# ruchikachavhan/diffusion-models-moe

Measured on AMD Instinct MI355X. Metric: images/sec SD-1.4 512² 50-step DDIM, expert mask on; 1→8 GPU scaling, higher is better.
Workload: dtype fp16; 1 GPU; SD-1.4 MoE-fied (relu, top-k 0.2, expert 20) + RemoveExperts skilled-expert mask, 512^2 (4x64x64 latents), 50 DDIM steps, CFG 7.5; prompts_per_gpu=8, global_batch=8, parallelism=dp1

## Files before the change

diffusion-models-moe_amd/csrc/gemm.hip:

```cpp
#include <array>
#include <utility>

#include "tune.h"
#include "../../include/sdmoe.h"
#include "gemm_kernel.h"

namespace {

enum TileId { T128x160, T64x160, T256x320, T256x160_42, T256x320_42, T128x320, T128x160_42, T64x320, T128x32, T128x64,
              T128x128, T64x128, NTILE };
struct TileShape { int bm, bn, wmw, wnw; };
constexpr TileShape kTile[NTILE] = {{128, 160, 2, 2}, {64, 160, 2, 2}, {256, 320, 2, 4}, {256, 160, 4, 2},
                                    {256, 320, 4, 2}, {128, 320, 2, 4}, {128, 160, 4, 2}, {64, 320, 2, 4},
                                    {128, 32, 2, 2},  {128, 64, 2, 2},  {128, 128, 2, 2}, {64, 128, 2, 2}};
struct Plan {
  int mode;
  int tile;
  int bk, stages;
  int ksplit;
  int kchunk;
  int kchunk2;
  int mfast;
};
struct TileRule { int tile, ks_want, stages_want; };
// ... 198 lines not shown
  const int pm = masked ? MODE_GEMM : mode;
  const TileRule r = choose_tile(pm, p);
  const int ksplit = plan_split(kTile[r.tile], pm, p, ws, ws_floats, r.ks_want);
  return tile_plan(mode, masked ? masked_tile(mode, r.tile, p) : r.tile, p, ksplit, r.stages_want);
}

bool plan_sets(int mode, const GemmParams& p, int rows_per_img, bool ws, long ws_floats, Plan* pl) {
  *pl = plan_launch(mode, p, ws, ws_floats);
  if (rows_per_img % kTile[pl->tile].bm == 0) return true;
  if (rows_per_img % 64) return false;
  const int tile = p.N % 160 == 0 ? T64x160 : T64x128;
  *pl = tile_plan(mode, tile, p, plan_split(kTile[tile], MODE_GEMM, p, ws, ws_floats, 0), 0);
  return true;
}

Plan plan_conv(const GemmParams& p, bool ws, long ws_floats) {
  Plan pl;
  if (plan_halo(p, ws, ws_floats, false, &pl)) return pl;
  return plan_launch(p.upsample ? MODE_CONV_UP : MODE_CONV, p, ws, ws_floats);
}

template <int MODE, int TILE>
int launch_kernel(const Plan& pl, const GemmParams& p, dim3 grid, hipStream_t s) {
  constexpr TileShape t = kTile[TILE];
  constexpr int NTH = 64 * t.wmw * t.wnw;
  if constexpr (!built(MODE, TILE)) return SDMOE_EUNSUP;
  else if constexpr (mode_halo(MODE)) gemm_kernel<t.bm, t.bn, t.wmw, t.wnw, MODE, 4, 32><<<grid, NTH, 0, s>>>(p);
  else if constexpr (!fits3(t, MODE)) gemm_kernel<t.bm, t.bn, t.wmw, t.wnw, MODE, 2, 64><<<grid, NTH, 0, s>>>(p);
  else if (pl.stages == 2) gemm_kernel<t.bm, t.bn, t.wmw, t.wnw, MODE, 2, 64><<<grid, NTH, 0, s>>>(p);
  else gemm_kernel<t.bm, t.bn, t.wmw, t.wnw, MODE, 3, 64><<<grid, NTH, 0, s>>>(p);
// ... 4 lines not shown
using LaunchFn = int (*)(const Plan&, const GemmParams&, dim3, hipStream_t);
template <int... KEY>
constexpr std::array<LaunchFn, sizeof...(KEY)> launch_table(std::integer_sequence<int, KEY...>) {
  return {{&launch_kernel<KEY / NTILE, KEY % NTILE>...}};
}
constexpr auto kLaunch = launch_table(std::make_integer_sequence<int, NMODE * NTILE>{});

int launch(const Plan& pl, GemmParams p, float* ws, hipStream_t s) {
  const TileShape& t = kTile[pl.tile];
  if (p.w_bstride && p.rows_per_batch % t.bm) return SDMOE_EUNSUP;
  if (p.image_set && p.rows_per_batch % t.bm) return SDMOE_EUNSUP;
  if (pl.ksplit > 1 && !ws) return SDMOE_EARG;
  p.ksplit = pl.ksplit; p.kchunk = pl.kchunk; p.kchunk2 = pl.kchunk2; p.mfast = pl.mfast;
  p.part = pl.ksplit > 1 ? ws : nullptr;
  p.diag = knob(KNOB_DIAG); p.res16 = knob(KNOB_RES16);
  const int direct = knob(KNOB_EPI_DIRECT);
  p.epi_direct = direct == 2 || (direct == 1 && p.R == nullptr);
  const dim3 grid(((p.M + t.bm - 1) / t.bm) * ((p.N + t.bn - 1) / t.bn) * pl.ksplit);
  if (const int st = kLaunch[pl.mode * NTILE + pl.tile](pl, p, grid, s)) return st;
  SDMOE_CHECK_LAUNCH();
  if (pl.ksplit > 1) {
    long nchunk = (long)p.M * (p.N / 8);
    int g = (int)((nchunk + 255) / 256);
    if (g > 2048) g = 2048;
    splitk_reduce_kernel<<<g, 256, 0, s>>>(p);
    SDMOE_CHECK_LAUNCH();
  }
  return SDMOE_OK;
}



// ... 435 lines not shown
                                long coladd_bstride, const void* R, long ldr, const void* X2, long ldx2, int Cin2,
                                void* Y, long ldy, int Cout, float* workspace, long workspace_floats, void* stream) {
  if (nimg == 0) return SDMOE_OK;
  if (!X || !gn_scale || !gn_shift || !Wt || !Y || nimg < 0 || H <= 0 || W <= 0 || Cout <= 0 || Cin2 < 0) return SDMOE_EARG;
  if (Cin % 64 || Cin2 % 64 || Cout % 8 || ldx % 8 || ldy % 8 || (R && ldr % 8) || (X2 && ldx2 % 8)) return SDMOE_ESHAPE;
  if ((X2 != nullptr) != (Cin2 > 0) || (X2 && R)) return SDMOE_EARG;
  GemmParams p{};
  conv_shape(p, nimg, H, W, Cin, Cin2, Cout, 1, 0, ACT_NONE);
  Plan pl;
  if (!plan_halo(p, workspace, workspace_floats, true, &pl)) return SDMOE_EUNSUP;
  if (const int st = fill_conv(p, X, ldx, Wt, bias, coladd, coladd_bstride, R, ldr, X2, ldx2, Y, ldy)) return st;
  p.gn_scale = gn_scale; p.gn_shift = gn_shift; p.gn_silu = silu;
  return launch(pl, p, workspace, (hipStream_t)stream);
}

extern "C" int sdmoe_groupnorm_apply(const void* X, long ldx, int nimg, int HW, int C, const float* scale,
                                     const float* shift, int silu, void* Y, long ldy, void* stream) {
  if (!X || !Y || !scale || !shift || nimg <= 0 || HW <= 0 || C <= 0) return SDMOE_EARG;
  if (C % 8 || ldx % 8 || ldy % 8) return SDMOE_ESHAPE;
  const long rows = (long)nimg * HW;
  gn_apply_kernel<<<grid_for(rows * (C / 8)), 256, 0, (hipStream_t)stream>>>(
      (const half_t*)X, ldx, HW, C, scale, shift, silu, (half_t*)Y, ldy, rows);
  SDMOE_CHECK_LAUNCH();
  return SDMOE_OK;
}

extern "C" int sdmoe_wmask_kmajor(const void* bits, long ldb, int N, int K, const int* perm, void* out, void* stream) {
  if (N == 0) return SDMOE_OK;
  if (!bits || !out || N < 0 || K <= 0) return SDMOE_EARG;
  if (K % 64 || ldb < K / 8) return SDMOE_ESHAPE;
// ... 16 lines not shown
```

diffusion-models-moe_amd/csrc/gemm_kernel.h:

```cpp
#pragma once
#include <type_traits>
#include <utility>
#include "common.h"

namespace {

typedef __attribute__((address_space(3))) void lds_void_t;

struct GemmParams {
  const half_t* A; long lda;
  const half_t* W; long ldw;
  const half_t* bias;
  const half_t* coladd; long coladd_bstride;
  const half_t* R; long ldr;
  half_t* C; long ldc;
  float* part;
  int M, N, K;
  int act;
  int rows_per_batch;
  int H, Wd, Cin, OH, OW, stride, upsample;
  int ksplit, kchunk;
  int kchunk2;
  int mfast;
  int a_bytes, w_bytes;
// ... 5 lines not shown
  const uint8_t* keep;
  int keep_bytes;
  const uint8_t* wmask;
  int wmask_bytes;
  const int* image_set;
  long wset_bytes;
  const float* ln_wsum;
  const float* ln_bias;
  float ln_eps;
  const half_t* A2; long lda2;
  int a2_bytes;
  long w_bstride;
  const float* colf; long colf_bstride;
  const half_t* gelu_tab;
  const float* gn_scale; const float* gn_shift; int gn_silu;
};

constexpr unsigned OOB = 0x80000000u;

SDMOE_DEV void bld16(__amdgpu_buffer_rsrc_t rs, char* lds_dst, unsigned voff, unsigned soff) {
  __builtin_amdgcn_raw_ptr_buffer_load_lds(rs, (lds_void_t*)lds_dst, 16, voff, soff, 0, 0);
}
SDMOE_DEV void wave_sync() {
  __builtin_amdgcn_fence(__ATOMIC_RELEASE, "wavefront");
  __builtin_amdgcn_wave_barrier();
  __builtin_amdgcn_fence(__ATOMIC_ACQUIRE, "wavefront");
}
template <int N>
SDMOE_DEV void vm_wait() { asm volatile("s_waitcnt vmcnt(%0)" ::"n"(N) : "memory"); }
SDMOE_DEV void vm_wait(int n) {
// ... 800 lines not shown
    for (int c = tid; c < BN; c += L.NT) {
      const bool ok = n0 + c < p.N;
      ln_col[c] = ok ? p.ln_wsum[n0 + c] : 0.f;
      ln_col[BN + c] = ok ? p.ln_bias[n0 + c] : 0.f;
    }
  }
  __syncthreads();
  constexpr int CPR = L.WN / 8;
  if (!G::GEGLU && p.act == ACT_NONE && (!p.R || p.res16 != 0)) {
    half4 b4[L.FN];
#pragma unroll
    for (int j = 0; j < L.FN; ++j) {
      const int n = nw + 16 * j + 4 * fg;
      b4[j] = (!G::LN && p.bias && n < p.N) ? *reinterpret_cast<const half4*>(p.bias + n) : (half4){0, 0, 0, 0};
    }
    if (!G::WKEEP && p.epi_direct) {
      const bool res = p.R != nullptr;
#pragma unroll
      for (int i = 0; i < L.FM; ++i) {
        __builtin_amdgcn_sched_barrier(0);
        const int m = mw + 16 * i + fr;
        const half_t* cap = (p.coladd && m < p.M) ? p.coladd + (long)(m / p.rows_per_batch) * p.coladd_bstride : nullptr;
        const float* cfp = (p.colf && m < p.M) ? p.colf + (long)(m / p.rows_per_batch) * p.colf_bstride : nullptr;
        float a = 0.f, c = 0.f;
        if constexpr (G::LN) {
          const int rl = wr * L.WM + 16 * i + fr;
          a = ln_row[2 * rl];
          c = ln_row[2 * rl + 1];
        }
        auto frag16 = [&](int j) -> uint2v {
          const int n = nw + 16 * j + 4 * fg;
          float4v v = acc[i][j];
// ... 22 lines not shown
          return __builtin_bit_cast(uint2v, y);
        };
#pragma unroll
        for (int j = 0; j + 1 < L.FN; j += 2) {
          const uint2v ya = frag16(j), yb = frag16(j + 1);
          const auto s0 = __builtin_amdgcn_permlane16_swap(ya[0], yb[0], false, false);
          const auto s1 = __builtin_amdgcn_permlane16_swap(ya[1], yb[1], false, false);
          const int n = nw + 16 * (j + (fg & 1)) + 8 * (fg >> 1);
          half8 o = __builtin_bit_cast(half8, (uint4v){s0[0], s1[0], s0[1], s1[1]});
          if (m < p.M && n < p.N) {
            if (res) {
              const half8 rr = *reinterpret_cast<const half8*>(p.R + (long)m * p.ldr + n);
#pragma unroll
              for (int r = 0; r < 8; ++r) o[r] = (half_t)((float)o[r] + (float)rr[r]);
            }
            if (p.diag & 8) asm volatile("" ::"v"(o));
            else *reinterpret_cast<half8*>(p.C + (long)m * p.ldc + n) = o;
          }
        }
        if constexpr (L.FN % 2) {
          const int n = nw + 16 * (L.FN - 1) + 4 * fg;
          half4 o = __builtin_bit_cast(half4, frag16(L.FN - 1));
          if (m < p.M && n < p.N) {
            if (res) {
              const half4 rr = *reinterpret_cast<const half4*>(p.R + (long)m * p.ldr + n);
#pragma unroll
              for (int r = 0; r < 4; ++r) o[r] = (half_t)((float)o[r] + (float)rr[r]);
            }
            if (p.diag & 8) asm volatile("" ::"v"(o));
            else *reinterpret_cast<half4*>(p.C + (long)m * p.ldc + n) = o;
          }
        }
      }
      return;
    }
    half_t* st = reinterpret_cast<half_t*>(smem) + wave * (L.WM / L.NPASS16) * L.RS16;
    constexpr int NCH16 = (L.WM / L.NPASS16) * CPR, NIT16 = (NCH16 + 63) / 64;
    const bool res = p.R != nullptr;
#pragma unroll
    for (int h = 0; h < L.NPASS16; ++h) {
      half8 rr[NIT16];
      if (res) {
#pragma unroll
        for (int it = 0; it < NIT16; ++it) {
          const int id = lane + 64 * it;
          const int r = id / CPR, c8 = id - r * CPR;
          const int m = mw + h * (L.WM / L.NPASS16) + r, n = nw + c8 * 8;
          rr[it] = (id < NCH16 && m < p.M && n < p.N) ? *reinterpret_cast<const half8*>(p.R + (long)m * p.ldr + n)
                                                      : (half8){0, 0, 0, 0, 0, 0, 0, 0};
        }
      }
#pragma unroll
      for (int i = 0; i < L.FM / L.NPASS16; ++i) {
// ... 35 lines not shown
          for (int r = 0; r < 4; ++r) y[r] = (half_t)v[r];
          *reinterpret_cast<half4*>(st + (16 * i + fr) * L.RS16 + 16 * j + 4 * fg) = y;
        }
      }
      wave_sync();
#pragma unroll
      for (int it = 0; it < NIT16; ++it) {
        const int id = lane + 64 * it;
        const int r = id / CPR, c8 = id - r * CPR;
        const int m = mw + h * (L.WM / L.NPASS16) + r, n = nw + c8 * 8;
        if (id >= NCH16 || m >= p.M || n >= p.N) continue;
        half8 o = *reinterpret_cast<const half8*>(st + r * L.RS16 + c8 * 8);
        if (res) {
#pragma unroll
          for (int j = 0; j < 8; ++j) o[j] = (half_t)((float)o[j] + (float)rr[it][j]);
        }
        if (p.diag & 8) asm volatile("" ::"v"(o));
        else *reinterpret_cast<half8*>(p.C + (long)m * p.ldc + n) = o;
      }
      wave_sync();
    }
    return;
  }
  if constexpr (G::GEGLU) {
    int lane_o = lane;
    asm volatile("" : "+v"(lane_o));
    const int fr_e = lane_o & 15, fg_e = lane_o >> 4;
    typedef _Float16 h2 __attribute__((ext_vector_type(2)));
    constexpr int NH = L.WN / 2;
    constexpr int FPP = L.FM % 2 == 0 ? 2 : 1;
    constexpr int RG = 16 * FPP;
    constexpr int GST = L.NW * 2 * RG * NH * 2;
    static_assert(NH % 8 == 0, "whole 16-B product chunks per row");
    static_assert(GST + L.NW * L.WN * 4 <= L.SMEM1, "GEGLU staging and bias must fit in the kernel's LDS");
    static_assert(GST + L.NW * L.WN * 4 == L.G_STAGING, "GEGLU staging size as the layout states it");
// ... 129 lines not shown
```

diffusion-models-moe_amd/csrc/norm.hip:

```cpp
#include "common.h"
#include "tune.h"
#include "../../include/sdmoe.h"

namespace {

constexpr int GN_SMALL_HW = 1024;
constexpr int GN_FUSED_HW = 256;

int gn_chunk_width(int C, int groups) {
  const int cpg = C / groups;
  int wc = cpg;
  while (wc % 8) wc += cpg;
  while (wc < 80 && C % (2 * wc) == 0 && 2 * wc <= 256) wc *= 2;
  return (wc <= 256 && wc / cpg <= 32 && C % wc == 0) ? wc : 0;
}

SDMOE_DEV float gn_ref(const half_t* g0, int cpg) {
  float s = 0.f;
#pragma unroll
  for (int j = 0; j < 8; ++j) s += (float)g0[(j * cpg) >> 3];
  return (float)(half_t)(s * 0.125f);
}

SDMOE_DEV void gn_accum8(const half8& v, const float (&rf)[8], float (&s1)[8], float (&s2)[8]) {
// ... 325 lines not shown
  const double n = (double)HW * cpg;
  const double ref = (double)gn_ref(X + (long)img * HW * ldx + g * cpg, cpg);
  const double m1 = a / n;
  double var = b / n - m1 * m1;
  if (var < 0) var = 0;
  const float mean = (float)(ref + m1);
  const float rstd = (float)(1.0 / sqrt(var + (double)eps));
  for (int c = lane; c < cpg; c += 64) {
    const int ch = g * cpg + c;
    const float sc = rstd * (float)gamma[ch];
    scale[(long)img * C + ch] = sc;
    shift[(long)img * C + ch] = (float)beta[ch] - mean * sc;
  }
}


template <int CPL>
__global__ __launch_bounds__(256) void layernorm_kernel(const half_t* __restrict__ X, long ldx, half_t* __restrict__ Y,
                                                        long ldy, int M, int C, const half_t* __restrict__ gamma,
                                                        const half_t* __restrict__ beta, float eps) {
  const int lane = threadIdx.x & 63, sub = lane & 7;
  const int row = blockIdx.x * (int)(blockDim.x >> 3) + (int)(threadIdx.x >> 3);
  const bool live = row < M;
  const half_t* xr = X + (long)(live ? row : 0) * ldx;
  half8 v[CPL];
#pragma unroll
  for (int i = 0; i < CPL; ++i) v[i] = *reinterpret_cast<const half8*>(xr + (sub + 8 * i) * 8);
  float s = 0.f;
#pragma unroll
  for (int i = 0; i < CPL; ++i)
// ... 54 lines not shown
  else
    gn_partial_kernel<1><<<dim3(S, nimg), 256, 0, s>>>((const half_t*)X, ldx, HW, C, groups, S, part);
  SDMOE_CHECK_LAUNCH();
  gn_finalize_kernel<<<dim3(groups, nimg), 64, 0, s>>>((const half_t*)X, ldx, HW, C, groups, S, part,
                                                       (const half_t*)gamma, (const half_t*)beta, eps, scale, shift);
  SDMOE_CHECK_LAUNCH();
  return SDMOE_OK;
}
}

extern "C" int sdmoe_groupnorm_stats(const void* X, long ldx, int nimg, int HW, int C, int groups,
                                     const void* gamma, const void* beta, float eps, float* scale, float* shift,
                                     float* workspace, long workspace_floats, void* stream) {
  return groupnorm_impl(X, ldx, nimg, HW, C, groups, gamma, beta, eps, scale, shift, workspace, workspace_floats,
                        stream);
}

extern "C" int sdmoe_groupnorm(const void* X, long ldx, int nimg, int HW, int C, int groups, const void* gamma,
                               const void* beta, float eps, int silu, void* Y, long ldy, float* scale, float* shift,
                               float* workspace, long workspace_floats, void* stream) {
  if (!Y || ldy % 8) return Y ? SDMOE_ESHAPE : SDMOE_EARG;
  if (knob(KNOB_GN_FUSED) && HW <= GN_FUSED_HW && X && gamma && beta && nimg > 0 && groups > 0 && C % groups == 0 &&
      C % 8 == 0 && ldx % 8 == 0 && groups <= 64) {
    const int wc = gn_chunk_width(C, groups);
    if (wc) {
      const int nchunk = C / wc;
      int S = (512 + nchunk * nimg - 1) / (nchunk * nimg);
      const int R = 256 / (wc / 8);
      if (S > HW / R) S = HW / R;
      if (S < 1) S = 1;
// ... 46 lines not shown
```

diffusion-models-moe_amd/sdmoe/_lib.py:

```python
from __future__ import annotations

import ctypes
import os

_HERE = os.path.dirname(os.path.abspath(__file__))
LIB_PATH = os.path.join(_HERE, "libsdmoe_hip.so")

_P = ctypes.c_void_p
_L = ctypes.c_long
_I = ctypes.c_int
_F = ctypes.c_float
_FP = ctypes.POINTER(ctypes.c_float)
_IP = ctypes.POINTER(ctypes.c_int)

SIGNATURES = {
    "sdmoe_linear": [_P, _L, _P, _L, _P, _P, _L, _I, _P, _L, _P, _L, _I, _I, _I, _I, _P, _L, _P],
    "sdmoe_conv3x3": [_P, _L, _I, _I, _I, _I, _P, _P, _P, _L, _P, _L, _P, _L, _I, _I, _I, _I, _P, _L, _P],
    "sdmoe_conv3x3_sc": [_P, _L, _I, _I, _I, _I, _P, _P, _P, _L, _P, _L, _I, _P, _L, _I, _I, _P, _L, _P],
    "sdmoe_conv3x3_gn": [_P, _L, _I, _I, _I, _I, _P, _P, _I, _P, _P, _P, _L, _P, _L, _P, _L, _I, _P, _L, _I, _P, _L,
                         _P],
    "sdmoe_groupnorm_apply": [_P, _L, _I, _I, _I, _P, _P, _I, _P, _L, _P],
    "sdmoe_mask_weight": [_P, _P, _L, _L, _P, _P],
    "sdmoe_groupnorm_stats": [_P, _L, _I, _I, _I, _I, _P, _P, _F, _P, _P, _P, _L, _P],
    "sdmoe_groupnorm": [_P, _L, _I, _I, _I, _I, _P, _P, _F, _I, _P, _L, _P, _P, _P, _L, _P],
    "sdmoe_gn_fold": [_P, _L, _I, _I, _P, _P, _P, _I, _P, _P, _P],
    "sdmoe_linear_per_image": [_P, _L, _P, _L, _L, _P, _L, _I, _P, _L, _P, _L, _I, _I, _I, _P, _L, _P],
    "sdmoe_layernorm": [_P, _L, _P, _L, _I, _I, _P, _P, _F, _P],
    "sdmoe_ln_fold": [_P, _L, _I, _I, _P, _P, _P, _P, _L, _P, _P, _P],
    "sdmoe_linear_ln": [_P, _L, _P, _L, _P, _P, _F, _P, _L, _I, _I, _I, _P],
    "sdmoe_linear_geglu_ln": [_P, _L, _P, _L, _P, _P, _F, _P, _L, _I, _I, _I, _I, _P, _L, _I, _P],
    "sdmoe_attention": [_P, _L, _P, _L, _P, _L, _P, _L, _I, _I, _I, _I, _I, _F, _P],
    "sdmoe_geglu_route": [_P, _L, _I, _I, _I, _I, _I, _P, _P, _P, _P, _P, _L, _P, _L, _P, _P, _P],
    "sdmoe_linear_geglu": [_P, _L, _P, _L, _P, _P, _L, _I, _I, _I, _I, _P, _L, _I, _P],
    "sdmoe_moe_topk_mask": [_P, _L, _I, _I, _I, _I, _I, _P, _L, _P, _P, _P],
    "sdmoe_moe_topk_keep": [_I, _I, _I, _I, _I, _P, _L, _P, _P, _P, _P],
# ... 107 lines not shown
```

diffusion-models-moe_amd/sdmoe/ops.py:

```python
from __future__ import annotations

import ctypes
import os

import torch

from . import _lib

ACT_NONE, ACT_SILU, ACT_GELU, ACT_RELU, ACT_QUICK_GELU = 0, 1, 2, 3, 4
ACT_BY_NAME = {"none": ACT_NONE, "silu": ACT_SILU, "gelu": ACT_GELU, "relu": ACT_RELU, "quick_gelu": ACT_QUICK_GELU}


_raw_stream = getattr(torch._C, "_cuda_getCurrentRawStream", None)
_cur_dev = getattr(torch._C, "_cuda_getDevice", None)


def _stream():
    if _raw_stream is not None and _cur_dev is not None:
        return _raw_stream(_cur_dev())
    return torch.cuda.current_stream().cuda_stream


def _ptr(t):
    return None if t is None else t.data_ptr()
# ... 347 lines not shown

def conv3x3_gn_launch(xp, ldx, nimg, H, W, Cin, w, bias, coladd, coladd_bstride, rp, ldr, out, op, ldy, Cout, gn,
                      sc=None):
    lib = _lib.load()
    ws = _workspace(out.device)
    x2p, ldx2, Cin2 = sc if sc is not None else (None, 0, 0)
    st = lib.sdmoe_conv3x3_gn(xp, ldx, nimg, H, W, Cin, gn[0].data_ptr(), gn[1].data_ptr(), int(bool(gn[2])),
                              _dev(w, "w"), _ptr(bias), _ptr(coladd), coladd_bstride, rp, ldr, x2p, ldx2, Cin2, op, ldy,
                              Cout, ws.data_ptr(), ws.numel(), _stream())
    if st == -3:
        return None
    _lib.check(st, "sdmoe_conv3x3_gn")
    return out


def conv3x3_launch(xp, ldx, nimg, H, W, Cin, w, bias, coladd, coladd_bstride, rp, ldr, out, op, ldy, Cout, stride,
                   upsample, act, sc=None):
    lib = _lib.load()
    ws = _workspace(out.device)
    if sc is not None:
        st = lib.sdmoe_conv3x3_sc(xp, ldx, nimg, H, W, Cin, _dev(w, "w"), _ptr(bias), _ptr(coladd), coladd_bstride,
                                  sc[0], sc[1], sc[2], op, ldy, Cout, act, ws.data_ptr(), ws.numel(), _stream())
        _lib.check(st, "sdmoe_conv3x3_sc")
        return out
    st = lib.sdmoe_conv3x3(xp, ldx, nimg, H, W, Cin, _dev(w, "w"), _ptr(bias), _ptr(coladd), coladd_bstride, rp, ldr,
                           op, ldy, Cout, stride, int(bool(upsample)), act, ws.data_ptr(), ws.numel(), _stream())
    _lib.check(st, "sdmoe_conv3x3")
    return out


# ... 585 lines not shown
```

diffusion-models-moe_amd/sdmoe/unet.py:

```python
from __future__ import annotations

import os

import torch
import torch.nn as nn
import torch.nn.functional as F

from . import ops
from .config import UNetConfig

CTX_LEN = 77
FUSED_GEGLU = True
FUSED_KEEP = True
FUSED_LN = os.environ.get("SDMOE_FUSED_LN", "1") != "0"
FUSED_LN_FFN = os.environ.get("SDMOE_FUSED_LN_FFN", "0") == "1"
FUSED_SC = os.environ.get("SDMOE_FUSED_SC", "1") != "0"
FUSED_GN = os.environ.get("SDMOE_FUSED_GN", "1") != "0"
GN_FOLD_MIN_HW = 1024
IN_PAD = 64
OUT_PAD = 8


def _buf(t):
    return nn.Parameter(t, requires_grad=False)


class LoRACompatibleLinear(nn.Module):

    def __init__(self, weight, bias=None):
        super().__init__()
        self.weight = _buf(weight)
        self.bias = None if bias is None else _buf(bias)
        self._sdmoe_deferred = 0
# ... 23 lines not shown
        self.weight = _buf(weight)
        self.bias = _buf(bias)
        self.stride = stride


class Norm(nn.Module):
    def __init__(self, weight, bias, eps, groups=None):
        super().__init__()
        self.weight = _buf(weight)
        self.bias = _buf(bias)
        self.eps = eps
        self.groups = groups

    def stats(self, x2d, nimg, HW):
        return ops.groupnorm_stats(x2d, nimg, HW, self.weight, self.bias, self.eps, self.groups)

    def normalize(self, x2d, nimg, HW, silu):
        return ops.groupnorm(x2d, nimg, HW, self.weight, self.bias, self.eps, self.groups, silu)


def act_code(fn):
    from_name = getattr(fn, "_sdmoe_act", None)
    if from_name is not None:
        return ops.ACT_BY_NAME[from_name]
    if fn is F.gelu or fn is torch.nn.functional.gelu:
        return ops.ACT_GELU
    if fn is F.relu or fn is torch.relu:
        return ops.ACT_RELU
    raise NotImplementedError(f"GEGLU activation {fn!r} has no HIP kernel (supported: gelu, relu)")

# ... 298 lines not shown
        n = ops.layernorm(hs, self.norm2.weight, self.norm2.bias, self.norm2.eps)
        hs = self.attn2.run(n, nimg, N, residual=hs, ctx2d=ctx2d)
        n = ops.layernorm(hs, self.norm3.weight, self.norm3.bias, self.norm3.eps)
        return self.ff.run(n, nimg, residual=hs)


class Transformer2DModel(nn.Module):

    def __init__(self, norm, proj_in, blocks, proj_out):
        super().__init__()
        self.norm = norm
        self.proj_in = proj_in
        self.transformer_blocks = nn.ModuleList(blocks)
        self.proj_out = proj_out

    def run(self, x, nimg, HW, ctx2d, out):
        pi = self.proj_in
        if FUSED_GN and HW >= GN_FOLD_MIN_HW and HW % 256 == 0 and x.shape[1] % 64 == 0 and not pi._forward_hooks:
            scale, shift = self.norm.stats(x, nimg, HW)
            wf, cb = ops.gn_fold(pi.weight, pi.bias, scale, shift)
            hs = ops.linear_per_image(x, wf, cb, HW)
        else:
            hs = pi.run(self.norm.normalize(x, nimg, HW, False))
        for blk in self.transformer_blocks:
            hs = blk.run(hs, nimg, HW, ctx2d)
        return self.proj_out.run(hs, residual=x, out=out)


class ResnetBlock2D(nn.Module):
    def __init__(self, norm1, conv1, temb_proj, norm2, conv2, shortcut):
        super().__init__()
        self.norm1, self.conv1, self.time_emb_proj, self.norm2, self.conv2 = norm1, conv1, temb_proj, norm2, conv2
        self.conv_shortcut = shortcut
        self.temb_slice = None
        self._sc_key = None
        self._sc_w = None

    def _conv2_with_shortcut(self):
        w2, b2, ws, bs = self.conv2.weight, self.conv2.bias, self.conv_shortcut.weight, self.conv_shortcut.bias
        key = tuple(None if t is None else (t.data_ptr(), t._version) for t in (w2, b2, ws, bs))
        if self._sc_key != key:
            b = sum(t.data.float() for t in (b2, bs) if t is not None)
            self._sc_w = (ops.conv_weight_with_shortcut(w2.data, ws.data),
                          None if isinstance(b, int) else b.half())
            self._sc_key = key
        return self._sc_w

    def run(self, x, nimg, H, W, temb_all, out):
        HW = H * W
        o, n = self.temb_slice
        bstride = temb_all.stride(0) if temb_all.shape[0] > 1 else 0
        cmid = self.conv1.weight.shape[0]
        if ops.conv_gn_fusable(H, W, x.shape[1], cmid):
            h = ops.conv3x3(x, nimg, H, W, self.conv1.weight, self.conv1.bias, coladd=temb_all[:, o:o + n],
                            coladd_bstride=bstride, gn=self.norm1.stats(x, nimg, HW) + (True,))
        else:
            xn = self.norm1.normalize(x, nimg, HW, True)
            h = ops.conv3x3(xn, nimg, H, W, self.conv1.weight, self.conv1.bias,
                            coladd=temb_all[:, o:o + n], coladd_bstride=bstride)
        gn2 = None
        hn = h
        if ops.conv_gn_fusable(H, W, cmid, self.conv2.weight.shape[0]):
            gn2 = self.norm2.stats(h, nimg, HW) + (True,)
        else:
            hn = self.norm2.normalize(h, nimg, HW, True)
        if self.conv_shortcut is not None and FUSED_SC and x.shape[1] % 64 == 0:
            w, b = self._conv2_with_shortcut()
            return ops.conv3x3(hn, nimg, H, W, w, b, shortcut=x, out=out, gn=gn2)
        res = x if self.conv_shortcut is None else self.conv_shortcut.run(x)
        return ops.conv3x3(hn, nimg, H, W, self.conv2.weight, self.conv2.bias, residual=res, out=out, gn=gn2)


class Sampler(nn.Module):
    def __init__(self, conv):
        super().__init__()
        self.conv = conv


class Block(nn.Module):

    def __init__(self, resnets, attentions=None, downsamplers=None, upsamplers=None):
        super().__init__()
        self.resnets = nn.ModuleList(resnets)
        if attentions:
            self.attentions = nn.ModuleList(attentions)
# ... 175 lines not shown
                cp = prev if j == 0 else cout
                cs = skip_in if j == L else cout
                buf = torch.empty((nimg * hh * hh, cp + cs), dtype=torch.float16, device=dev)
                up_in.append((buf, cp, hh))
            prev = cout
        nskip = len(up_in)

        def skip_slot(k):
            buf, cp, _ = up_in[nskip - 1 - k]
            return buf[:, cp:]

        def new(rows, c):
            return torch.empty((rows, c), dtype=torch.float16, device=dev)

        k = 0
        h = ops.conv3x3(x_in, nimg, H, W, self.conv_in.weight, self.conv_in.bias, out=skip_slot(k))
        k += 1
        hh = H
        for i, blk in enumerate(self.down_blocks):
            rows = nimg * hh * hh
            for j in range(L):
                if blk.attentions is not None:
                    r = blk.resnets[j].run(h, nimg, hh, hh, temb_all, out=new(rows, ch[i]))
                    h = blk.attentions[j].run(r, nimg, hh * hh, ctx2d, out=skip_slot(k))
                else:
                    h = blk.resnets[j].run(h, nimg, hh, hh, temb_all, out=skip_slot(k))
                k += 1
            if hasattr(blk, "downsamplers"):
                c = blk.downsamplers[0].conv
                h = ops.conv3x3(h, nimg, hh, hh, c.weight, c.bias, stride=2, out=skip_slot(k))
                k += 1
                hh //= 2

        rows = nimg * hh * hh
        mb = self.mid_block
        r = mb.resnets[0].run(h, nimg, hh, hh, temb_all, out=new(rows, ch[-1]))
        a = mb.attentions[0].run(r, nimg, hh * hh, ctx2d, out=new(rows, ch[-1]))
        buf0, cp0, _ = up_in[0]
        mb.resnets[1].run(a, nimg, hh, hh, temb_all, out=buf0[:, :cp0])

        idx = 0
        final = None
        for i, blk in enumerate(self.up_blocks):
            cout = rev[i]
            for j in range(L + 1):
                inp, cp, hh = up_in[idx]
                rows = nimg * hh * hh
                last_in_block = j == L
                has_up = hasattr(blk, "upsamplers")
                if not last_in_block:
                    nb, ncp, _ = up_in[idx + 1]
                    dest = nb[:, :ncp]
                elif has_up or i == nblk - 1:
                    dest = new(rows, cout)
                if blk.attentions is not None:
                    r = blk.resnets[j].run(inp, nimg, hh, hh, temb_all, out=new(rows, cout))
                    o = blk.attentions[j].run(r, nimg, hh * hh, ctx2d, out=dest)
                else:
                    o = blk.resnets[j].run(inp, nimg, hh, hh, temb_all, out=dest)
                idx += 1
                if last_in_block:
                    if has_up:
                        nb, ncp, _ = up_in[idx]
                        c = blk.upsamplers[0].conv
                        ops.conv3x3(o, nimg, hh, hh, c.weight, c.bias, upsample=True, out=nb[:, :ncp])
                    else:
                        final = o

        fn = self.conv_norm_out.normalize(final, nimg, H * W, True)
        if out is None:
            out = new(nimg * H * W, OUT_PAD)
        return ops.conv3x3(fn, nimg, H, W, self.conv_out.weight, self.conv_out.bias, out=out)
# ... 12 lines not shown
```

include/sdmoe.h:

```cpp
#ifndef SDMOE_H
#define SDMOE_H

#ifdef __cplusplus
extern "C" {
#endif

#define SDMOE_ACT_NONE 0
#define SDMOE_ACT_SILU 1
#define SDMOE_ACT_GELU 2
#define SDMOE_ACT_RELU 3
#define SDMOE_ACT_QUICK_GELU 4

const char* sdmoe_version(void);

int sdmoe_linear(const void* A, long lda, const void* W, long ldw, const void* bias, const void* coladd,
                 long coladd_bstride, int rows_per_batch, const void* R, long ldr, void* C, long ldc, int M, int N,
                 int K, int act, float* workspace, long workspace_floats, void* stream);

int sdmoe_conv3x3(const void* X, long ldx, int nimg, int H, int W, int Cin, const void* Wt, const void* bias,
                  const void* coladd, long coladd_bstride, const void* R, long ldr, void* Y, long ldy, int Cout,
                  int stride, int upsample, int act, float* workspace, long workspace_floats, void* stream);

int sdmoe_conv3x3_sc(const void* X, long ldx, int nimg, int H, int W, int Cin, const void* Wt, const void* bias,
                     const void* coladd, long coladd_bstride, const void* X2, long ldx2, int Cin2, void* Y, long ldy,
                     int Cout, int act, float* workspace, long workspace_floats, void* stream);

int sdmoe_conv3x3_gn(const void* X, long ldx, int nimg, int H, int W, int Cin, const float* gn_scale,
                     const float* gn_shift, int silu, const void* Wt, const void* bias, const void* coladd,
                     long coladd_bstride, const void* R, long ldr, const void* X2, long ldx2, int Cin2, void* Y,
                     long ldy, int Cout, float* workspace, long workspace_floats, void* stream);
int sdmoe_groupnorm_apply(const void* X, long ldx, int nimg, int HW, int C, const float* scale, const float* shift,
                          int silu, void* Y, long ldy, void* stream);

int sdmoe_mask_weight(const void* W, const void* bits, long N, long K, void* Wm, void* stream);

int sdmoe_groupnorm_stats(const void* X, long ldx, int nimg, int HW, int C, int groups, const void* gamma,
                          const void* beta, float eps, float* scale, float* shift, float* workspace,
                          long workspace_floats, void* stream);

int sdmoe_groupnorm(const void* X, long ldx, int nimg, int HW, int C, int groups, const void* gamma, const void* beta,
                    float eps, int silu, void* Y, long ldy, float* scale, float* shift, float* workspace,
                    long workspace_floats, void* stream);

int sdmoe_gn_fold(const void* W, long ldw, int N, int K, const void* bias, const float* scale, const float* shift,
                  int nimg, void* Wf, float* colbias, void* stream);
// ... 115 lines not shown
```

Baseline: 9.622 images/s.

## Emit GroupNorm partial statistics from conv epilogue to skip separate stats pass

Adds a path where the 64x64, 320-channel halo conv kernel computes per-slice, per-group shifted sums and sums of squares in its epilogue and writes them to a small partials buffer. A new finalize kernel merges the slices Welford-style into GroupNorm scale and shift, and the UNet resnet, attention and conv_in paths consume these partials instead of rereading the activation for a separate groupnorm_stats pass. It is on by default behind an env flag. In exchange the conv epilogue does extra shared-memory work and reductions, which may add register or LDS pressure to the hottest conv.

Result: no change. 9.611 images/s (-0.1%).

```diff
diff --git a/diffusion-models-moe_amd/csrc/gemm.hip b/diffusion-models-moe_amd/csrc/gemm.hip
--- a/diffusion-models-moe_amd/csrc/gemm.hip
+++ b/diffusion-models-moe_amd/csrc/gemm.hip
@@ -236,6 +236,17 @@
   return true;
 }
 
+bool plan_epi_direct(const GemmParams& p) {
+  const int direct = knob(KNOB_EPI_DIRECT);
+  return direct == 2 || (direct == 1 && p.R == nullptr);
+}
+
+int plan_gn_slices(const Plan& pl, const GemmParams& p) {
+  if (pl.mode != MODE_CONVH64 || pl.tile != T256x320 || pl.ksplit != 1 || p.N != 320 || p.act != ACT_NONE || p.colf)
+    return 0;
+  return 2 * (p.H * p.Wd / 256);
+}
+
 Plan plan_conv(const GemmParams& p, bool ws, long ws_floats) {
   Plan pl;
   if (plan_halo(p, ws, ws_floats, false, &pl)) return pl;
@@ -270,8 +281,7 @@
   p.ksplit = pl.ksplit; p.kchunk = pl.kchunk; p.kchunk2 = pl.kchunk2; p.mfast = pl.mfast;
   p.part = pl.ksplit > 1 ? ws : nullptr;
   p.diag = knob(KNOB_DIAG); p.res16 = knob(KNOB_RES16);
-  const int direct = knob(KNOB_EPI_DIRECT);
-  p.epi_direct = direct == 2 || (direct == 1 && p.R == nullptr);
+  p.epi_direct = plan_epi_direct(p);
   const dim3 grid(((p.M + t.bm - 1) / t.bm) * ((p.N + t.bn - 1) / t.bn) * pl.ksplit);
   if (const int st = kLaunch[pl.mode * NTILE + pl.tile](pl, p, grid, s)) return st;
   SDMOE_CHECK_LAUNCH();
@@ -737,6 +747,51 @@
   return launch(pl, p, workspace, (hipStream_t)stream);
 }
 
+static bool plan_conv_part(const GemmParams& p, bool gn, bool ws, long ws_floats, Plan* pl) {
+  if (gn) {
+    if (!plan_halo(p, ws, ws_floats, true, pl)) return false;
+  } else {
+    *pl = plan_conv(p, ws, ws_floats);
+  }
+  return plan_gn_slices(*pl, p) > 0;
+}
+
+extern "C" int sdmoe_conv_gn_slices(int nimg, int H, int W, int Cin, int Cin2, int Cout, int has_residual, int gn,
+                                    long workspace_floats) {
+  if (nimg <= 0 || H <= 0 || W <= 0 || Cin <= 0 || Cin2 < 0 || Cout <= 0 || workspace_floats < 0 ||
+      (Cin2 && has_residual) || Cin % 64 || Cin2 % 64 || Cout % 8)
+    return 0;
+  GemmParams p{};
+  conv_shape(p, nimg, H, W, Cin, Cin2, Cout, 1, 0, ACT_NONE);
+  p.R = has_residual ? reinterpret_cast<const half_t*>(&p) : nullptr;
+  Plan pl;
+  if (!plan_conv_part(p, gn != 0, workspace_floats > 0, workspace_floats, &pl)) return 0;
+  return plan_gn_slices(pl, p);
+}
+
+extern "C" int sdmoe_conv3x3_part(const void* X, long ldx, int nimg, int H, int W, int Cin, const float* gn_scale,
+                                  const float* gn_shift, int silu, const void* Wt, const void* bias, const void* coladd,
+                                  long coladd_bstride, const void* R, long ldr, const void* X2, long ldx2, int Cin2,
+                                  void* Y, long ldy, int Cout, float* workspace, long workspace_floats, float* part,
+                                  long part_floats, void* stream) {
+  if (nimg == 0) return SDMOE_OK;
+  if (!X || !Wt || !Y || !part || nimg < 0 || H <= 0 || W <= 0 || Cout <= 0 || Cin2 < 0 ||
+      (gn_scale != nullptr) != (gn_shift != nullptr))
+    return SDMOE_EARG;
+  if (Cin % 64 || Cin2 % 64 || Cout % 8 || ldx % 8 || ldy % 8 || (R && ldr % 8) || (X2 && ldx2 % 8)) return SDMOE_ESHAPE;
+  if ((X2 != nullptr) != (Cin2 > 0) || (X2 && R)) return SDMOE_EARG;
+  GemmParams p{};
+  conv_shape(p, nimg, H, W, Cin, Cin2, Cout, 1, 0, ACT_NONE);
+  p.R = (const half_t*)R;
+  Plan pl;
+  if (!plan_conv_part(p, gn_scale != nullptr, workspace, workspace_floats, &pl)) return SDMOE_EUNSUP;
+  if ((long)nimg * 32 * plan_gn_slices(pl, p) * 3 > part_floats) return SDMOE_EARG;
+  if (const int st = fill_conv(p, X, ldx, Wt, bias, coladd, coladd_bstride, R, ldr, X2, ldx2, Y, ldy)) return st;
+  p.gn_scale = gn_scale; p.gn_shift = gn_shift; p.gn_silu = silu;
+  p.gn_part = part;
+  return launch(pl, p, workspace, (hipStream_t)stream);
+}
+
 extern "C" int sdmoe_groupnorm_apply(const void* X, long ldx, int nimg, int HW, int C, const float* scale,
                                      const float* shift, int silu, void* Y, long ldy, void* stream) {
   if (!X || !Y || !scale || !shift || nimg <= 0 || HW <= 0 || C <= 0) return SDMOE_EARG;
diff --git a/diffusion-models-moe_amd/csrc/gemm_kernel.h b/diffusion-models-moe_amd/csrc/gemm_kernel.h
--- a/diffusion-models-moe_amd/csrc/gemm_kernel.h
+++ b/diffusion-models-moe_amd/csrc/gemm_kernel.h
@@ -43,6 +43,7 @@
   const float* colf; long colf_bstride;
   const half_t* gelu_tab;
   const float* gn_scale; const float* gn_shift; int gn_silu;
+  float* gn_part;
 };
 
 constexpr unsigned OOB = 0x80000000u;
@@ -873,8 +874,74 @@
       const int n = nw + 16 * j + 4 * fg;
       b4[j] = (!G::LN && p.bias && n < p.N) ? *reinterpret_cast<const half4*>(p.bias + n) : (half4){0, 0, 0, 0};
     }
+    constexpr bool GNP = MODE == MODE_CONVH64 && BM == 256 && BN == 320 && WMW == 2 && WNW == 4;
+    auto gn_emit = [&](const float* pair_sum, const float* group_ref) {
+      if (lane < 8) {
+        float s1 = 0.f, s2 = 0.f;
+#pragma unroll
+        for (int t = 0; t < 5; ++t) {
+          s1 += pair_sum[5 * lane + t];
+          s2 += pair_sum[40 + 5 * lane + t];
+        }
+        const int pix = p.H * L.HW_, img = m0 / pix, tiles = pix / BM;
+        const int slice = 2 * ((m0 - img * pix) / BM) + wr;
+        float* rec = p.gn_part + (((long)img * 32 + wc * 8 + lane) * (2 * tiles) + slice) * 3;
+        rec[0] = group_ref[lane];
+        rec[1] = s1;
+        rec[2] = s2;
+      }
+    };
     if (!G::WKEEP && p.epi_direct) {
       const bool res = p.R != nullptr;
+      bool gnp = false;
+      half_t* const g_row = reinterpret_cast<half_t*>(smem + wave * 1024);
+      float* const g_ref = reinterpret_cast<float*>(smem + wave * 1024 + 256);
+      float* const g_sum = reinterpret_cast<float*>(smem + wave * 1024 + 512);
+      char* const g_acc = smem + 8192 + wave * 8192 + lane * 16;
+      auto g_slot = [&](int v) -> float4v& { return *reinterpret_cast<float4v*>(g_acc + v * 1024); };
+      auto g_pair = [&](int k) {
+        return k < 8 ? 16 * (k >> 2) + 8 * (fg & 1) + 4 * (fg >> 1) + (k & 3) : 32 + 2 * fg + (k - 8);
+      };
+      if constexpr (GNP) {
+        gnp = p.gn_part != nullptr;
+        if (gnp) {
+          const half_t* cap0 = p.coladd ? p.coladd + (long)(mw / p.rows_per_batch) * p.coladd_bstride : nullptr;
+#pragma unroll
+          for (int j = 0; j < L.FN; ++j) {
+            const int n = nw + 16 * j + 4 * fg;
+            float4v v = acc[0][j];
+#pragma unroll
+            for (int r = 0; r < 4; ++r) v[r] += (float)b4[j][r];
+            if (cap0) {
+              const half4 cc = *reinterpret_cast<const half4*>(cap0 + n);
+#pragma unroll
+              for (int r = 0; r < 4; ++r) v[r] += (float)cc[r];
+            }
+            half4 y;
+#pragma unroll
+            for (int r = 0; r < 4; ++r) y[r] = (half_t)v[r];
+            if (res) {
+              const half4 rr = *reinterpret_cast<const half4*>(p.R + (long)mw * p.ldr + n);
+#pragma unroll
+              for (int r = 0; r < 4; ++r) y[r] = (half_t)((float)y[r] + (float)rr[r]);
+            }
+            if (fr == 0) *reinterpret_cast<half4*>(g_row + 16 * j + 4 * fg) = y;
+          }
+          wave_sync();
+          if (lane < 8) {
+            float s = 0.f;
+#pragma unroll
+            for (int j = 0; j < 8; ++j) s += (float)g_row[lane * 10 + ((j * 10) >> 3)];
+            g_ref[lane] = (float)(half_t)(s * 0.125f);
+          }
+          wave_sync();
+          g_slot(5) = (float4v){g_ref[g_pair(0) / 5], g_ref[g_pair(1) / 5], g_ref[g_pair(2) / 5], g_ref[g_pair(3) / 5]};
+          g_slot(6) = (float4v){g_ref[g_pair(4) / 5], g_ref[g_pair(5) / 5], g_ref[g_pair(6) / 5], g_ref[g_pair(7) / 5]};
+          g_slot(7) = (float4v){g_ref[g_pair(8) / 5], g_ref[g_pair(9) / 5], 0.f, 0.f};
+#pragma unroll
+          for (int v = 0; v < 5; ++v) g_slot(v) = (float4v){0.f, 0.f, 0.f, 0.f};
+        }
+      }
 #pragma unroll
       for (int i = 0; i < L.FM; ++i) {
         __builtin_amdgcn_sched_barrier(0);
@@ -927,6 +994,20 @@
 #pragma unroll
               for (int r = 0; r < 8; ++r) o[r] = (half_t)((float)o[r] + (float)rr[r]);
             }
+            if constexpr (GNP) {
+              if (gnp) {
+                const float4v rf = g_slot(5 + j / 2);
+                float4v a1 = g_slot(j), a2 = g_slot(j + 1);
+#pragma unroll
+                for (int r = 0; r < 8; ++r) {
+                  const float d = (float)o[r] - rf[r / 2];
+                  a1[r / 2] += d;
+                  a2[r / 2] = __builtin_fmaf(d, d, a2[r / 2]);
+                }
+                g_slot(j) = a1;
+                g_slot(j + 1) = a2;
+              }
+            }
             if (p.diag & 8) asm volatile("" ::"v"(o));
             else *reinterpret_cast<half8*>(p.C + (long)m * p.ldc + n) = o;
           }
@@ -940,9 +1021,43 @@
 #pragma unroll
               for (int r = 0; r < 4; ++r) o[r] = (half_t)((float)o[r] + (float)rr[r]);
             }
+            if constexpr (GNP) {
+              if (gnp) {
+                const float4v rf = g_slot(7);
+                float4v a = g_slot(4);
+#pragma unroll
+                for (int r = 0; r < 4; ++r) {
+                  const float d = (float)o[r] - rf[r / 2];
+                  a[r / 2] += d;
+                  a[2 + r / 2] = __builtin_fmaf(d, d, a[2 + r / 2]);
+                }
+                g_slot(4) = a;
+              }
+            }
             if (p.diag & 8) asm volatile("" ::"v"(o));
             else *reinterpret_cast<half4*>(p.C + (long)m * p.ldc + n) = o;
           }
+        }
+      }
+      if constexpr (GNP) {
+        if (gnp) {
+          const float4v v0 = g_slot(0), v1 = g_slot(1), v2 = g_slot(2), v3 = g_slot(3), v4 = g_slot(4);
+          float gs1[10] = {v0[0], v0[1], v0[2], v0[3], v2[0], v2[1], v2[2], v2[3], v4[0], v4[1]};
+          float gs2[10] = {v1[0], v1[1], v1[2], v1[3], v3[0], v3[1], v3[2], v3[3], v4[2], v4[3]};
+#pragma unroll
+          for (int k = 0; k < 10; ++k) {
+#pragma unroll
+            for (int x = 1; x < 16; x <<= 1) {
+              gs1[k] += __shfl_xor(gs1[k], x, 64);
+              gs2[k] += __shfl_xor(gs2[k], x, 64);
+            }
+            if (fr == 0) {
+              g_sum[g_pair(k)] = gs1[k];
+              g_sum[40 + g_pair(k)] = gs2[k];
+            }
+          }
+          wave_sync();
+          gn_emit(g_sum, g_ref);
         }
       }
       return;
@@ -950,6 +1065,11 @@
     half_t* st = reinterpret_cast<half_t*>(smem) + wave * (L.WM / L.NPASS16) * L.RS16;
     constexpr int NCH16 = (L.WM / L.NPASS16) * CPR, NIT16 = (NCH16 + 63) / 64;
     const bool res = p.R != nullptr;
+    bool gnq = false;
+    float q_s1 = 0.f, q_s2 = 0.f, q_ref = 0.f;
+    float* const q_ref8 = reinterpret_cast<float*>(smem + 96 * 1024 + wave * 1024);
+    float* const q_sum = q_ref8 + 8;
+    if constexpr (GNP) gnq = p.gn_part != nullptr;
 #pragma unroll
     for (int h = 0; h < L.NPASS16; ++h) {
       half8 rr[NIT16];
@@ -1015,11 +1135,52 @@
         if (res) {
 #pragma unroll
           for (int j = 0; j < 8; ++j) o[j] = (half_t)((float)o[j] + (float)rr[it][j]);
+          if constexpr (GNP) {
+            if (gnq) *reinterpret_cast<half8*>(st + r * L.RS16 + c8 * 8) = o;
+          }
         }
         if (p.diag & 8) asm volatile("" ::"v"(o));
         else *reinterpret_cast<half8*>(p.C + (long)m * p.ldc + n) = o;
       }
+      if constexpr (GNP) {
+        if (gnq) {
+          static_assert(!GNP || L.NW * (L.WM / L.NPASS16) * L.RS16 * 2 <= 96 * 1024, "staging below the sums");
+          wave_sync();
+          if (h == 0) {
+            if (lane < 8) {
+              float s = 0.f;
+#pragma unroll
+              for (int j = 0; j < 8; ++j) s += (float)st[lane * 10 + ((j * 10) >> 3)];
+              q_ref8[lane] = (float)(half_t)(s * 0.125f);
+            }
+            wave_sync();
+            q_ref = q_ref8[(lane < 40 ? lane : 0) / 5];
+          }
+          if (lane < 40) {
+#pragma unroll 8
+            for (int r = 0; r < L.WM / L.NPASS16; ++r) {
+              typedef _Float16 h2 __attribute__((ext_vector_type(2)));
+              const h2 x = *reinterpret_cast<const h2*>(st + r * L.RS16 + 2 * lane);
+              const float d0 = (float)x[0] - q_ref, d1 = (float)x[1] - q_ref;
+              q_s1 += d0;
+              q_s2 = __builtin_fmaf(d0, d0, q_s2);
+              q_s1 += d1;
+              q_s2 = __builtin_fmaf(d1, d1, q_s2);
+            }
+          }
+        }
+      }
       wave_sync();
+    }
+    if constexpr (GNP) {
+      if (gnq) {
+        if (lane < 40) {
+          q_sum[lane] = q_s1;
+          q_sum[40 + lane] = q_s2;
+        }
+        wave_sync();
+        gn_emit(q_sum, q_ref8);
+      }
     }
     return;
   }
diff --git a/diffusion-models-moe_amd/csrc/norm.hip b/diffusion-models-moe_amd/csrc/norm.hip
--- a/diffusion-models-moe_amd/csrc/norm.hip
+++ b/diffusion-models-moe_amd/csrc/norm.hip
@@ -363,6 +363,44 @@
   }
 }
 
+__global__ __launch_bounds__(64) void gn_finalize_slices_kernel(const float* __restrict__ part, int C, int G, int S,
+                                                                double n, const half_t* __restrict__ gamma,
+                                                                const half_t* __restrict__ beta, float eps,
+                                                                float* __restrict__ scale, float* __restrict__ shift) {
+  const int g = blockIdx.x, img = blockIdx.y, lane = threadIdx.x;
+  const int cpg = C / G;
+  double cnt = 0.0, mean = 0.0, m2 = 0.0;
+  if (lane < S) {
+    const float* r = part + (((long)img * G + g) * S + lane) * 3;
+    const double ref = r[0], s1 = r[1], s2 = r[2];
+    cnt = n;
+    mean = ref + s1 / n;
+    m2 = s2 - s1 * s1 / n;
+    if (m2 < 0) m2 = 0;
+  }
+#pragma unroll
+  for (int o = 1; o < 64; o <<= 1) {
+    const double cb = __shfl_down(cnt, o, 64), mb = __shfl_down(mean, o, 64), qb = __shfl_down(m2, o, 64);
+    if ((lane & (2 * o - 1)) == 0 && cb > 0) {
+      const double tot = cnt + cb, d = mb - mean;
+      mean += d * (cb / tot);
+      m2 += qb + d * d * (cnt * cb / tot);
+      cnt = tot;
+    }
+  }
+  cnt = __shfl(cnt, 0, 64);
+  mean = __shfl(mean, 0, 64);
+  m2 = __shfl(m2, 0, 64);
+  const float meanf = (float)mean;
+  const float rstd = (float)(1.0 / sqrt(m2 / cnt + (double)eps));
+  for (int c = lane; c < cpg; c += 64) {
+    const int ch = g * cpg + c;
+    const float sc = rstd * (float)gamma[ch];
+    scale[(long)img * C + ch] = sc;
+    shift[(long)img * C + ch] = (float)beta[ch] - meanf * sc;
+  }
+}
+
 
 template <int CPL>
 __global__ __launch_bounds__(256) void layernorm_kernel(const half_t* __restrict__ X, long ldx, half_t* __restrict__ Y,
@@ -447,6 +485,19 @@
                                      float* workspace, long workspace_floats, void* stream) {
   return groupnorm_impl(X, ldx, nimg, HW, C, groups, gamma, beta, eps, scale, shift, workspace, workspace_floats,
                         stream);
+}
+
+extern "C" int sdmoe_groupnorm_finalize_slices(const float* part, int nimg, int C, int groups, int S,
+                                               int rows_per_slice, const void* gamma, const void* beta, float eps,
+                                               float* scale, float* shift, void* stream) {
+  if (!part || !gamma || !beta || !scale || !shift || nimg <= 0 || groups <= 0 || S <= 0 || rows_per_slice <= 0)
+    return SDMOE_EARG;
+  if (C <= 0 || C % groups || S > 64) return SDMOE_ESHAPE;
+  gn_finalize_slices_kernel<<<dim3(groups, nimg), 64, 0, (hipStream_t)stream>>>(
+      part, C, groups, S, (double)rows_per_slice * (C / groups), (const half_t*)gamma, (const half_t*)beta, eps, scale,
+      shift);
+  SDMOE_CHECK_LAUNCH();
+  return SDMOE_OK;
 }
 
 extern "C" int sdmoe_groupnorm(const void* X, long ldx, int nimg, int HW, int C, int groups, const void* gamma,
diff --git a/diffusion-models-moe_amd/sdmoe/_lib.py b/diffusion-models-moe_amd/sdmoe/_lib.py
--- a/diffusion-models-moe_amd/sdmoe/_lib.py
+++ b/diffusion-models-moe_amd/sdmoe/_lib.py
@@ -19,6 +19,10 @@
     "sdmoe_conv3x3_sc": [_P, _L, _I, _I, _I, _I, _P, _P, _P, _L, _P, _L, _I, _P, _L, _I, _I, _P, _L, _P],
     "sdmoe_conv3x3_gn": [_P, _L, _I, _I, _I, _I, _P, _P, _I, _P, _P, _P, _L, _P, _L, _P, _L, _I, _P, _L, _I, _P, _L,
                          _P],
+    "sdmoe_conv_gn_slices": [_I, _I, _I, _I, _I, _I, _I, _I, _L],
+    "sdmoe_conv3x3_part": [_P, _L, _I, _I, _I, _I, _P, _P, _I, _P, _P, _P, _L, _P, _L, _P, _L, _I, _P, _L, _I, _P, _L,
+                           _P, _L, _P],
+    "sdmoe_groupnorm_finalize_slices": [_P, _I, _I, _I, _I, _I, _P, _P, _F, _P, _P, _P],
     "sdmoe_groupnorm_apply": [_P, _L, _I, _I, _I, _P, _P, _I, _P, _L, _P],
     "sdmoe_mask_weight": [_P, _P, _L, _L, _P, _P],
     "sdmoe_groupnorm_stats": [_P, _L, _I, _I, _I, _I, _P, _P, _F, _P, _P, _P, _L, _P],
diff --git a/diffusion-models-moe_amd/sdmoe/ops.py b/diffusion-models-moe_amd/sdmoe/ops.py
--- a/diffusion-models-moe_amd/sdmoe/ops.py
+++ b/diffusion-models-moe_amd/sdmoe/ops.py
@@ -385,6 +385,74 @@
     return out
 
 
+def conv_gn_slices(nimg, H, W, Cin, Cout, *, Cin2=0, residual=False, gn=False, workspace_floats=WS_FLOATS):
+    lib = _lib.load()
+    if not _lib.has(lib, "sdmoe_conv_gn_slices"):
+        return 0
+    return lib.sdmoe_conv_gn_slices(nimg, H, W, Cin, Cin2, Cout, int(bool(residual)), int(bool(gn)), workspace_floats)
+
+
+def conv3x3_partials(x, nimg, H, W, w, bias=None, *, out=None, residual=None, coladd=None, coladd_bstride=0, gn=None,
+                     shortcut=None, part=None):
+    lib = _lib.load()
+    Cin, Cout = x.shape[1], w.shape[0]
+    Cin2 = 0 if shortcut is None else shortcut.shape[1]
+    S = 0
+    if gn is None or conv_gn_fusable(H, W, Cin, Cout):
+        S = conv_gn_slices(nimg, H, W, Cin, Cout, Cin2=Cin2, residual=residual is not None, gn=gn is not None,
+                           workspace_floats=_workspace(x.device).numel())
+    if S == 0:
+        return conv3x3(x, nimg, H, W, w, bias, out=out, residual=residual, coladd=coladd,
+                       coladd_bstride=coladd_bstride, gn=gn, shortcut=shortcut), None
+    xp, ldx = _rows(x, "x")
+    if x.shape[0] != nimg * H * W:
+        raise ValueError("conv3x3: rows != nimg*H*W")
+    x2p, ldx2 = (None, 0)
+    if shortcut is not None:
+        x2p, ldx2 = _rows(shortcut, "shortcut")
+        if w.dim() != 2 or w.shape[1] != 9 * Cin + Cin2 or residual is not None or shortcut.shape[0] != x.shape[0]:
+            raise ValueError(f"conv3x3: weight {tuple(w.shape)} is not [Cout, 9*{Cin} + {Cin2}], or a residual was "
+                             "given, or the shortcut's rows differ")
+    elif w.dim() != 5 or tuple(w.shape[1:]) != (Cin // 64, 3, 3, 64):
+        raise ValueError(f"conv3x3: weight {tuple(w.shape)} is not the [Cout, Cin/64, 3, 3, 64] layout for Cin={Cin}")
+    gsc = gsh = None
+    silu = False
+    if gn is not None:
+        sc, sh, silu = gn
+        if tuple(sc.shape) != (nimg, Cin) or sc.dtype != torch.float32 or tuple(sh.shape) != (nimg, Cin):
+            raise ValueError("conv3x3: gn scale / shift must be fp32 [nimg, Cin]")
+        gsc, gsh = _dev(sc, "gn scale", torch.float32), _dev(sh, "gn shift", torch.float32)
+    if out is None:
+        out = torch.empty((nimg * H * W, Cout), dtype=torch.float16, device=x.device)
+    op, ldy = _rows(out, "out")
+    rp, ldr = (None, 0) if residual is None else _rows(residual, "residual")
+    if part is None:
+        part = torch.empty((nimg, 32, S, 3), dtype=torch.float32, device=x.device)
+    elif tuple(part.shape) != (nimg, 32, S, 3):
+        raise ValueError(f"conv3x3: partials buffer {tuple(part.shape)} is not {(nimg, 32, S, 3)}")
+    ws = _workspace(out.device)
+    st = lib.sdmoe_conv3x3_part(xp, ldx, nimg, H, W, Cin, gsc, gsh, int(bool(silu)), _dev(w, "w"), _ptr(bias),
+                                _ptr(coladd), coladd_bstride, rp, ldr, x2p, ldx2, Cin2, op, ldy, Cout, ws.data_ptr(),
+                                ws.numel(), _dev(part, "part", torch.float32), part.numel(), _stream())
+    _lib.check(st, "sdmoe_conv3x3_part")
+    return out, part
+
+
+def groupnorm_stats_from(part, nimg, HW, C, gamma, beta, eps, groups=32):
+    lib = _lib.load()
+    S = part.shape[2]
+    if tuple(part.shape) != (nimg, groups, S, 3) or HW % S:
+        raise ValueError(f"groupnorm_stats_from: partials {tuple(part.shape)} do not match {nimg} images of {groups} "
+                         f"groups over {HW} rows")
+    scale = torch.empty((nimg, C), dtype=torch.float32, device=part.device)
+    shift = torch.empty((nimg, C), dtype=torch.float32, device=part.device)
+    st = lib.sdmoe_groupnorm_finalize_slices(_dev(part, "part", torch.float32), nimg, C, groups, S, HW // S,
+                                             _dev(gamma, "gamma"), _dev(beta, "beta"), float(eps), scale.data_ptr(),
+                                             shift.data_ptr(), _stream())
+    _lib.check(st, "sdmoe_groupnorm_finalize_slices")
+    return scale, shift
+
+
 def conv3x3_launch(xp, ldx, nimg, H, W, Cin, w, bias, coladd, coladd_bstride, rp, ldr, out, op, ldy, Cout, stride,
                    upsample, act, sc=None):
     lib = _lib.load()
diff --git a/diffusion-models-moe_amd/sdmoe/unet.py b/diffusion-models-moe_amd/sdmoe/unet.py
--- a/diffusion-models-moe_amd/sdmoe/unet.py
+++ b/diffusion-models-moe_amd/sdmoe/unet.py
@@ -17,6 +17,7 @@
 FUSED_SC = os.environ.get("SDMOE_FUSED_SC", "1") != "0"
 FUSED_GN = os.environ.get("SDMOE_FUSED_GN", "1") != "0"
 GN_FOLD_MIN_HW = 1024
+CONV_GN_PARTIALS = os.environ.get("SDMOE_CONV_GN_PARTIALS", "1") != "0"
 IN_PAD = 64
 OUT_PAD = 8
 
@@ -70,6 +71,13 @@
 
     def stats(self, x2d, nimg, HW):
         return ops.groupnorm_stats(x2d, nimg, HW, self.weight, self.bias, self.eps, self.groups)
+
+    def accepts(self, part):
+        return part is not None and part.shape[1] == self.groups and self.weight.shape[0] == 10 * self.groups
+
+    def stats_from(self, part, nimg, HW):
+        return ops.groupnorm_stats_from(part, nimg, HW, self.weight.shape[0], self.weight, self.bias, self.eps,
+                                        self.groups)
 
     def normalize(self, x2d, nimg, HW, silu):
         return ops.groupnorm(x2d, nimg, HW, self.weight, self.bias, self.eps, self.groups, silu)
@@ -398,10 +406,13 @@
         self.transformer_blocks = nn.ModuleList(blocks)
         self.proj_out = proj_out
 
-    def run(self, x, nimg, HW, ctx2d, out):
+    def run(self, x, nimg, HW, ctx2d, out, x_part=None):
         pi = self.proj_in
         if FUSED_GN and HW >= GN_FOLD_MIN_HW and HW % 256 == 0 and x.shape[1] % 64 == 0 and not pi._forward_hooks:
-            scale, shift = self.norm.stats(x, nimg, HW)
+            if self.norm.accepts(x_part) and not self.norm._forward_hooks:
+                scale, shift = self.norm.stats_from(x_part, nimg, HW)
+            else:
+                scale, shift = self.norm.stats(x, nimg, HW)
             wf, cb = ops.gn_fold(pi.weight, pi.bias, scale, shift)
             hs = ops.linear_per_image(x, wf, cb, HW)
         else:
@@ -430,14 +441,23 @@
             self._sc_key = key
         return self._sc_w
 
-    def run(self, x, nimg, H, W, temb_all, out):
+    def run(self, x, nimg, H, W, temb_all, out, x_part=None, emit=False):
         HW = H * W
+        hooked = any(m is not None and m._forward_hooks
+                     for m in (self.norm1, self.conv1, self.norm2, self.conv2, self.conv_shortcut))
+        partials = CONV_GN_PARTIALS and not hooked
+        if not partials:
+            x_part = None
         o, n = self.temb_slice
         bstride = temb_all.stride(0) if temb_all.shape[0] > 1 else 0
         cmid = self.conv1.weight.shape[0]
+        h_part = None
         if ops.conv_gn_fusable(H, W, x.shape[1], cmid):
-            h = ops.conv3x3(x, nimg, H, W, self.conv1.weight, self.conv1.bias, coladd=temb_all[:, o:o + n],
-                            coladd_bstride=bstride, gn=self.norm1.stats(x, nimg, HW) + (True,))
+            gn1 = (self.norm1.stats_from(x_part, nimg, HW) if self.norm1.accepts(x_part)
+                   else self.norm1.stats(x, nimg, HW)) + (True,)
+            conv = ops.conv3x3_partials if partials else _conv3x3_plain
+            h, h_part = conv(x, nimg, H, W, self.conv1.weight, self.conv1.bias, coladd=temb_all[:, o:o + n],
+                             coladd_bstride=bstride, gn=gn1)
         else:
             xn = self.norm1.normalize(x, nimg, HW, True)
             h = ops.conv3x3(xn, nimg, H, W, self.conv1.weight, self.conv1.bias,
@@ -445,14 +465,22 @@
         gn2 = None
         hn = h
         if ops.conv_gn_fusable(H, W, cmid, self.conv2.weight.shape[0]):
-            gn2 = self.norm2.stats(h, nimg, HW) + (True,)
+            gn2 = (self.norm2.stats_from(h_part, nimg, HW) if self.norm2.accepts(h_part)
+                   else self.norm2.stats(h, nimg, HW)) + (True,)
         else:
             hn = self.norm2.normalize(h, nimg, HW, True)
+        conv2 = ops.conv3x3_partials if partials and emit else _conv3x3_plain
         if self.conv_shortcut is not None and FUSED_SC and x.shape[1] % 64 == 0:
             w, b = self._conv2_with_shortcut()
-            return ops.conv3x3(hn, nimg, H, W, w, b, shortcut=x, out=out, gn=gn2)
-        res = x if self.conv_shortcut is None else self.conv_shortcut.run(x)
-        return ops.conv3x3(hn, nimg, H, W, self.conv2.weight, self.conv2.bias, residual=res, out=out, gn=gn2)
+            y = conv2(hn, nimg, H, W, w, b, shortcut=x, out=out, gn=gn2)
+        else:
+            res = x if self.conv_shortcut is None else self.conv_shortcut.run(x)
+            y = conv2(hn, nimg, H, W, self.conv2.weight, self.conv2.bias, residual=res, out=out, gn=gn2)
+        return y if emit else y[0]
+
+
+def _conv3x3_plain(*a, **kw):
+    return ops.conv3x3(*a, **kw), None
 
 
 class Sampler(nn.Module):
@@ -658,17 +686,22 @@
             return torch.empty((rows, c), dtype=torch.float16, device=dev)
 
         k = 0
-        h = ops.conv3x3(x_in, nimg, H, W, self.conv_in.weight, self.conv_in.bias, out=skip_slot(k))
+        if CONV_GN_PARTIALS and not self.conv_in._forward_hooks:
+            h, h_part = ops.conv3x3_partials(x_in, nimg, H, W, self.conv_in.weight, self.conv_in.bias, out=skip_slot(k))
+        else:
+            h, h_part = ops.conv3x3(x_in, nimg, H, W, self.conv_in.weight, self.conv_in.bias, out=skip_slot(k)), None
         k += 1
         hh = H
         for i, blk in enumerate(self.down_blocks):
             rows = nimg * hh * hh
             for j in range(L):
                 if blk.attentions is not None:
-                    r = blk.resnets[j].run(h, nimg, hh, hh, temb_all, out=new(rows, ch[i]))
-                    h = blk.attentions[j].run(r, nimg, hh * hh, ctx2d, out=skip_slot(k))
+                    r, r_part = blk.resnets[j].run(h, nimg, hh, hh, temb_all, out=new(rows, ch[i]), x_part=h_part,
+                                                   emit=True)
+                    h = blk.attentions[j].run(r, nimg, hh * hh, ctx2d, out=skip_slot(k), x_part=r_part)
                 else:
-                    h = blk.resnets[j].run(h, nimg, hh, hh, temb_all, out=skip_slot(k))
+                    h = blk.resnets[j].run(h, nimg, hh, hh, temb_all, out=skip_slot(k), x_part=h_part)
+                h_part = None
                 k += 1
             if hasattr(blk, "downsamplers"):
                 c = blk.downsamplers[0].conv
@@ -698,8 +731,8 @@
                 elif has_up or i == nblk - 1:
                     dest = new(rows, cout)
                 if blk.attentions is not None:
-                    r = blk.resnets[j].run(inp, nimg, hh, hh, temb_all, out=new(rows, cout))
-                    o = blk.attentions[j].run(r, nimg, hh * hh, ctx2d, out=dest)
+                    r, r_part = blk.resnets[j].run(inp, nimg, hh, hh, temb_all, out=new(rows, cout), emit=True)
+                    o = blk.attentions[j].run(r, nimg, hh * hh, ctx2d, out=dest, x_part=r_part)
                 else:
                     o = blk.resnets[j].run(inp, nimg, hh, hh, temb_all, out=dest)
                 idx += 1
diff --git a/include/sdmoe.h b/include/sdmoe.h
--- a/include/sdmoe.h
+++ b/include/sdmoe.h
@@ -29,6 +29,17 @@
                      const float* gn_shift, int silu, const void* Wt, const void* bias, const void* coladd,
                      long coladd_bstride, const void* R, long ldr, const void* X2, long ldx2, int Cin2, void* Y,
                      long ldy, int Cout, float* workspace, long workspace_floats, void* stream);
+
+int sdmoe_conv_gn_slices(int nimg, int H, int W, int Cin, int Cin2, int Cout, int has_residual, int gn,
+                         long workspace_floats);
+int sdmoe_conv3x3_part(const void* X, long ldx, int nimg, int H, int W, int Cin, const float* gn_scale,
+                       const float* gn_shift, int silu, const void* Wt, const void* bias, const void* coladd,
+                       long coladd_bstride, const void* R, long ldr, const void* X2, long ldx2, int Cin2, void* Y,
+                       long ldy, int Cout, float* workspace, long workspace_floats, float* part, long part_floats,
+                       void* stream);
+int sdmoe_groupnorm_finalize_slices(const float* part, int nimg, int C, int groups, int S, int rows_per_slice,
+                                    const void* gamma, const void* beta, float eps, float* scale, float* shift,
+                                    void* stream);
 int sdmoe_groupnorm_apply(const void* X, long ldx, int nimg, int HW, int C, const float* scale, const float* shift,
                           int silu, void* Y, long ldy, void* stream);
 
```
